# jackie840129/FedFR

Measured on AMD Instinct MI355X. Metric: images/sec (iresnet100+CosFace train step, bs=128/GPU, 112x112), higher is better.
Workload: dtype fp16; 1 GPU; iresnet100 + CosFace(s=30,m=0.4) + dense 1000-class cosine head, full train step (fwd+bwd+momentum-SGD), batch 128/GPU, 112x112 synthetic faces, random-init weights, fp16 activations/weights with fp32 accumulate + fp32 master weights, fp32 head; global_batch=128, parallelism=1 client per GPU (FedAvg), dp1, clients=1

## Files before the change

### fedfr_amd/csrc/gemm_nt_glds.hip

```cpp
#include "nt_epilogue.h"

#ifndef NT_GLDS_NS
#define NT_GLDS_NS 4
#endif
namespace {
template <int N_>
__device__ __forceinline__ void wait_vmcnt() {
  asm volatile("s_waitcnt vmcnt(%0)" ::"n"(N_) : "memory");
}

template <int BM, int BN, int WM, int WN, int NS, bool CONV>
__global__ __launch_bounds__(64 * WM * WN) void gemm_nt_glds_kernel(GemmNT p_) {
  GemmNT p = p_;
  if (p.par_on == 2) {
    const int cls = 3 - (int)blockIdx.z;
    p.par_h = cls >> 1; p.par_w = cls & 1;
    p.ksteps_total = (1 + p.par_h) * (1 + p.par_w) * p.cpt;
    p.ksteps_per_split = p.ksteps_total;
  }
  constexpr int NW = WM * WN, NT = 64 * NW;
  constexpr int TM = BM / WM / 16, TN = BN / WN / 16;
  constexpr int A_BYTES = BM * 128, B_BYTES = BN * 128, STAGE = A_BYTES + B_BYTES;
  constexpr int AP = (BM / 8) / NW, BP = (BN / 8) / NW, PER = AP + BP;
  constexpr int NRD = TM + TN, NM = TM * TN;
  static_assert((BM / 8) % NW == 0 && (BN / 8) % NW == 0 && NS >= 3 && NS <= 5 && AP >= 1 && BP >= 1, "tile geometry");
  typedef __attribute__((address_space(3))) void* lds_ptr_t;
  extern __shared__ __attribute__((aligned(1024))) unsigned char smem[];

  const int tid = threadIdx.x, lane = tid & 63;
  const int wave = __builtin_amdgcn_readfirstlane(tid >> 6);
  const int wm = wave / WN, wn = wave % WN;
  const int lid = xcd_remap(blockIdx.x, gridDim.x);
  const int bn = lid % p.nbn, bm = lid / p.nbn;
  const int split = blockIdx.y;
  const int m0 = bm * BM, n0 = bn * BN;
  const int kt0 = split * p.ksteps_per_split;
  const int kt1 = min(kt0 + p.ksteps_per_split, p.ksteps_total);

  const int prow = lane >> 3, pch = (lane & 7) ^ prow;
  constexpr unsigned OOB = 0xfffffff0u;
  int a_hb[AP], a_wb[AP];
  unsigned a_base[AP];
  bool a_ok[AP];
#pragma unroll
  for (int j = 0; j < AP; ++j) {
    const int m = m0 + (j * NW + wave) * 8 + prow;
    a_ok[j] = m < p.M;
    if (CONV) {
      const int mm = a_ok[j] ? m : 0;
      const int hw = p.Ho * p.Wo;
      const int img = mm / hw, rem = mm - img * hw;
      int ho = rem / p.Wo, wo = rem - ho * p.Wo;
      if (p.par_on) {
        ho = 2 * ho + p.par_h;
        wo = 2 * wo + p.par_w;
      }
      a_hb[j] = ho * p.stride - p.pad;
      a_wb[j] = wo * p.stride - p.pad;
      a_base[j] = ((unsigned)(img * p.H * p.W) * (unsigned)p.C + (unsigned)(pch * 8)) * 2u;
    } else {
      a_hb[j] = a_wb[j] = 0;
      a_base[j] = ((unsigned)(a_ok[j] ? m : 0) * (unsigned)p.lda + (unsigned)(pch * 8)) * 2u;
    }
  }
  unsigned b_base[BP];
  bool b_ok[BP];
#pragma unroll
  for (int j = 0; j < BP; ++j) {
    const int n = n0 + (j * NW + wave) * 8 + prow;
    b_ok[j] = n < p.N;
    b_base[j] = ((unsigned)(b_ok[j] ? n : 0) * (unsigned)p.K + (unsigned)(pch * 8)) * 2u;
  }
  int kti = kt0;
  int tap = kt0 / p.cpt, cc = kt0 - tap * p.cpt;
  int r = tap / p.S, s = tap - r * p.S;
  const int s0 = p.par_on ? 1 - p.par_w : 0, tstep = p.par_on ? 2 : 1;
  if (p.par_on) {
    const int nS = 1 + p.par_w;
    r = (1 - p.par_h) + 2 * (tap / nS);
    s = s0 + 2 * (tap % nS);
  }
  const __amdgpu_buffer_rsrc_t rsA = make_rsrc(p.A, p.a_bytes), rsB = make_rsrc(p.B, p.b_bytes);
  const int upm = p.up - 1, ups = p.up >> 1;
  const unsigned rowB = (unsigned)(p.W * p.C * 2), pixB = (unsigned)(p.C * 2);
  auto issue = [&](int slot) {
    unsigned char* sA = smem + slot * STAGE;
    unsigned char* sB = sA + A_BYTES;
    const bool live = kti < kt1;
    const unsigned kA = (unsigned)(CONV ? cc * 128 : kti * 128);
    const bool klive = live & (CONV | (kti * 64 + pch * 8 < p.K));
#pragma unroll
    for (int j = 0; j < AP; ++j) {
      bool ok = klive & a_ok[j];
      unsigned off = a_base[j] + kA;
      if (CONV) {
        int hp = a_hb[j] + r, wp = a_wb[j] + s;
        ok = ok & (((hp | wp) & upm) == 0);
        hp >>= ups;
        wp >>= ups;
        ok = ok & ((unsigned)hp < (unsigned)p.H) & ((unsigned)wp < (unsigned)p.W);
        off += __umul24((unsigned)hp, rowB) + __umul24((unsigned)wp, pixB);
      }
      __builtin_amdgcn_raw_ptr_buffer_load_lds(rsA, (lds_ptr_t)(sA + (j * NW + wave) * 1024), 16, (int)(ok ? off : OOB), 0, 0, 0);
    }
    const unsigned kB = (unsigned)(CONV ? ((r * p.S + s) * p.cpt + cc) * 128 : kti * 128);
#pragma unroll
    for (int j = 0; j < BP; ++j)
      __builtin_amdgcn_raw_ptr_buffer_load_lds(rsB, (lds_ptr_t)(sB + (j * NW + wave) * 1024), 16, (int)((klive & b_ok[j]) ? b_base[j] + kB : OOB), 0, 0, 0);
    ++kti;
    cc += 1;
    const bool wc = cc == p.cpt;
    cc = wc ? 0 : cc;
    s += wc ? tstep : 0;
    const bool ws = s >= p.S;
    s = ws ? s0 : s;
    r += ws ? tstep : 0;
  };

  const int l15 = lane & 15, lg = lane >> 4;
  int a_addr[TM], b_addr[TN];
#pragma unroll
  for (int mi = 0; mi < TM; ++mi) {
    const int row = wm * (BM / WM) + mi * 16 + l15;
    a_addr[mi] = row * 128 + ((lg ^ (row & 7)) << 4);
  }
#pragma unroll
  for (int ni = 0; ni < TN; ++ni) {
    const int row = wn * (BN / WN) + ni * 16 + l15;
    b_addr[ni] = A_BYTES + row * 128 + ((lg ^ (row & 7)) << 4);
  }
  f32x4_t acc[TN][TM];
#pragma unroll
  for (int a = 0; a < TN; ++a)
#pragma unroll
    for (int b = 0; b < TM; ++b) acc[a][b] = (f32x4_t){0.f, 0.f, 0.f, 0.f};
  bf16x8_t f0a[TM], f0b[TN], f1a[TM], f1b[TN];
  auto read_frags = [&](bf16x8_t (&fa)[TM], bf16x8_t (&fb)[TN], const unsigned char* st, int ks) {
#pragma unroll
    for (int ni = 0; ni < TN; ++ni) fb[ni] = *reinterpret_cast<const bf16x8_t*>(st + (b_addr[ni] ^ (ks * 64)));
#pragma unroll
    for (int mi = 0; mi < TM; ++mi) fa[mi] = *reinterpret_cast<const bf16x8_t*>(st + (a_addr[mi] ^ (ks * 64)));
  };
  auto mfma_all = [&](const bf16x8_t (&fa)[TM], const bf16x8_t (&fb)[TN]) {
#pragma unroll
    for (int ni = 0; ni < TN; ++ni)
#pragma unroll
      for (int mi = 0; mi < TM; ++mi) acc[ni][mi] = MFMA16(fb[ni], fa[mi], acc[ni][mi]);
  };

#pragma unroll
  for (int i = 0; i < NS - 1; ++i) issue(i);
  wait_vmcnt<(NS - 2) * PER>();
  __builtin_amdgcn_s_barrier();
  read_frags(f0a, f0b, smem, 0);
  int slot = 0;
  for (int kt = kt0; kt < kt1; ++kt) {
    const unsigned char* cur = smem + slot * STAGE;
    const int nslot = slot + 1 == NS ? 0 : slot + 1, fslot = slot == 0 ? NS - 1 : slot - 1;
    read_frags(f1a, f1b, cur, 1);
    mfma_all(f0a, f0b);
#pragma unroll
    for (int i = 0; i < NRD; ++i) {
      __builtin_amdgcn_sched_group_barrier(0x008, (NM / NRD) > 0 ? (NM / NRD) : 1, 0);
      __builtin_amdgcn_sched_group_barrier(0x100, 1, 0);
    }
    __builtin_amdgcn_sched_barrier(0);
    wait_vmcnt<(NS - 3) * PER>();
    __builtin_amdgcn_s_barrier();
    __builtin_amdgcn_sched_barrier(0);
    read_frags(f0a, f0b, smem + nslot * STAGE, 0);
    issue(fslot);
    mfma_all(f1a, f1b);
    constexpr int NE = NRD > PER ? NRD : PER, MP2 = (NM / NE) > 0 ? (NM / NE) : 1;
#pragma unroll
    for (int i = 0; i < NE; ++i) {
      __builtin_amdgcn_sched_group_barrier(0x008, MP2, 0);
      if (i < NRD) __builtin_amdgcn_sched_group_barrier(0x100, 1, 0);
      if (i < PER) __builtin_amdgcn_sched_group_barrier(0x020, 1, 0);
    }
    __builtin_amdgcn_sched_barrier(0);
    slot = nslot;
  }
  wait_vmcnt<0>();
  __syncthreads();
  nt_epilogue<BM, BN, WM, WN, NT>(p, acc, smem, bm, m0, n0, split, wm, wn, tid, lane);
}

template <int BM, int BN, int WM, int WN, int NS, bool CONV>
int launch_impl2(GemmNT p, int splits, int slot, hipStream_t st) {
  const int nbm = ceil_div(p.M, BM);
  p.nbn = ceil_div(p.N, BN);
  p.ksteps_per_split = ceil_div(p.ksteps_total, splits);
  FEDFR_REQUIRE(ceil_div(p.ksteps_total, p.ksteps_per_split) == splits, "gemm_nt_glds: splits=%d leaves an empty split (ksteps=%d)", splits,
                p.ksteps_total);
  constexpr size_t kRing = (size_t)NS * (BM + BN) * 128, kEpi = (size_t)BM * (BN * 2 + 16);
  constexpr size_t lds = kRing > kEpi ? kRing : kEpi;
  static PerDeviceOnce attr_once;
  attr_once.run([&] {
    hipFuncSetAttribute(reinterpret_cast<const void*>(&gemm_nt_glds_kernel<BM, BN, WM, WN, NS, CONV>), hipFuncAttributeMaxDynamicSharedMemorySize, (int)lds);
  });
  const dim3 grid(nbm * p.nbn, splits, p.par_on == 2 ? 4 : 1);
  ProfScope prof(slot, 2.0 * p.M * p.N * (p.par_on == 2 ? 64.0 * 9 * p.cpt : p.par_on ? 64.0 * p.ksteps_total : (double)p.K), st, gemm_nt_alg_bytes(p, splits));
  hipLaunchKernelGGL((gemm_nt_glds_kernel<BM, BN, WM, WN, NS, CONV>), grid, dim3(64 * WM * WN), lds, st, p);
  FEDFR_LAUNCH_CHECK("gemm_nt_glds");
  return FEDFR_OK;
}
template <int BM, int BN, int WM, int WN, int NS>
int launch_impl(const GemmNT& p, int splits, int slot, hipStream_t st) {
  if (p.mode == 1) {
    FEDFR_REQUIRE((long long)p.W * p.C * 2 < (1 << 24) && p.H < (1 << 15), "gemm_nt_glds: image row too large for the 24-bit address multiplies");
    return launch_impl2<BM, BN, WM, WN, NS, true>(p, splits, slot, st);
  }
  return launch_impl2<BM, BN, WM, WN, NS, false>(p, splits, slot, st);
}
}

int g_nt_glds = 4;

bool gemm_nt_glds_applies(const GemmNT& p, int BM, int splits) {
  const bool pays = (g_nt_glds & 8) || (!p.par_on && ceil_div(p.ksteps_total, splits) >= 16);
  return (g_nt_glds & 7) > 0 && p.N > 64 && (BM == 128 || BM == 64) && pays && !p.bpart && !p.esc && !p.eadd && !p.Cb2;
}

int launch_nt_glds(const GemmNT& p, int BM, int splits, int slot, hipStream_t st) {
  FEDFR_REQUIRE(gemm_nt_glds_applies(p, BM, splits), "gemm_nt_glds: unsupported problem");
  const int v = g_nt_glds & 7;
  const bool up = v >= 3 && BM == 64 && (!p.stats || ceil_div(p.M, 64) == 2 * ceil_div(p.M, 128));
  if (BM == 128 || up) return (v & 1) == 0 ? launch_impl<128, 128, 2, 4, NT_GLDS_NS>(p, splits, slot, st) : launch_impl<128, 128, 2, 2, 4>(p, splits, slot, st);
  return launch_impl<64, 128, 1, 4, 3>(p, splits, slot, st);
}
```

Measured before the change: 8402 images/sec.

## Hoist implicit-GEMM conv gather address math to once per filter tap

Adds a tap-stepped variant of the conv gather GEMM kernel, templated on channel-chunks-per-tap (1,2,4,8). Per-row spatial coordinates and validity are computed once, and the per-tap voffset and validity are recomputed only when the filter tap advances. Between tap changes each k-step just adds the chunk offset, which removes integer address arithmetic and predicate work from the inner loop. The cost is more template instantiations and extra registers held across the loop, which could lower occupancy.

Measured after the change: 8423 images/sec, median of 6. About the same (+0.2%).

```diff
diff --git a/fedfr_amd/csrc/gemm_nt_glds.hip b/fedfr_amd/csrc/gemm_nt_glds.hip
--- a/fedfr_amd/csrc/gemm_nt_glds.hip
+++ b/fedfr_amd/csrc/gemm_nt_glds.hip
@@ -1,7 +1,11 @@
 #include "nt_epilogue.h"
+#include "nt_gather_plan.h"
 
 #ifndef NT_GLDS_NS
 #define NT_GLDS_NS 4
+#endif
+#ifndef NT_GLDS_TAPSTEP
+#define NT_GLDS_TAPSTEP 1
 #endif
 namespace {
 template <int N_>
@@ -9,8 +13,9 @@
   asm volatile("s_waitcnt vmcnt(%0)" ::"n"(N_) : "memory");
 }
 
-template <int BM, int BN, int WM, int WN, int NS, bool CONV>
+template <int BM, int BN, int WM, int WN, int NS, bool CONV, int CPT>
 __global__ __launch_bounds__(64 * WM * WN) void gemm_nt_glds_kernel(GemmNT p_) {
+  static_assert(CPT == 0 || CONV, "the tap-stepped plan is the conv gather's");
   GemmNT p = p_;
   if (p.par_on == 2) {
     const int cls = 3 - (int)blockIdx.z;
@@ -116,6 +121,39 @@
     s = ws ? s0 : s;
     r += ws ? tstep : 0;
   };
+  const NtPlanGeom pg = nt_plan_geom(p.H, p.W, p.C, p.S, p.up, p.cpt, p.par_on, p.par_w);
+  NtPlanRow prw[AP];
+  unsigned voff_tap[AP], kB_tap = 0;
+  bool ok_tap[AP];
+  auto plan_tap = [&]() {
+#pragma unroll
+    for (int j = 0; j < AP; ++j) nt_plan_tap(pg, prw[j], r, s, voff_tap[j], ok_tap[j]);
+    kB_tap = nt_plan_weight_tap(pg, r, s);
+  };
+  if constexpr (CPT > 0) {
+#pragma unroll
+    for (int j = 0; j < AP; ++j)
+      prw[j] = nt_plan_row(m0 + (j * NW + wave) * 8 + prow, p.M, p.Ho, p.Wo, p.H, p.W, p.C, p.stride, p.pad, p.par_on, p.par_h, p.par_w, pch);
+    nt_plan_tap_first(pg, p.par_on, p.par_h, p.par_w, kt0 / CPT, r, s);
+    plan_tap();
+  }
+  auto issue_tap = [&](int slot, int ci) {
+    unsigned char* sA = smem + slot * STAGE;
+    unsigned char* sB = sA + A_BYTES;
+    const bool live = kti < kt1;
+#pragma unroll
+    for (int j = 0; j < AP; ++j)
+      __builtin_amdgcn_raw_ptr_buffer_load_lds(rsA, (lds_ptr_t)(sA + (j * NW + wave) * 1024), 16, (int)nt_plan_voffset(voff_tap[j], ok_tap[j], live, ci), 0, 0, 0);
+    const unsigned kB = kB_tap + (unsigned)ci * 128u;
+#pragma unroll
+    for (int j = 0; j < BP; ++j)
+      __builtin_amdgcn_raw_ptr_buffer_load_lds(rsB, (lds_ptr_t)(sB + (j * NW + wave) * 1024), 16, (int)((live & b_ok[j]) ? b_base[j] + kB : OOB), 0, 0, 0);
+    ++kti;
+    if (ci == CPT - 1) {
+      nt_plan_tap_next(pg, r, s);
+      plan_tap();
+    }
+  };
 
   const int l15 = lane & 15, lg = lane >> 4;
   int a_addr[TM], b_addr[TN];
@@ -149,12 +187,15 @@
   };
 
 #pragma unroll
-  for (int i = 0; i < NS - 1; ++i) issue(i);
+  for (int i = 0; i < NS - 1; ++i) {
+    if constexpr (CPT > 0) issue_tap(i, i % CPT);
+    else issue(i);
+  }
   wait_vmcnt<(NS - 2) * PER>();
   __builtin_amdgcn_s_barrier();
   read_frags(f0a, f0b, smem, 0);
   int slot = 0;
-  for (int kt = kt0; kt < kt1; ++kt) {
+  auto kstep = [&](auto&& issue_next) {
     const unsigned char* cur = smem + slot * STAGE;
     const int nslot = slot + 1 == NS ? 0 : slot + 1, fslot = slot == 0 ? NS - 1 : slot - 1;
     read_frags(f1a, f1b, cur, 1);
@@ -169,7 +210,7 @@
     __builtin_amdgcn_s_barrier();
     __builtin_amdgcn_sched_barrier(0);
     read_frags(f0a, f0b, smem + nslot * STAGE, 0);
-    issue(fslot);
+    issue_next(fslot);
     mfma_all(f1a, f1b);
     constexpr int NE = NRD > PER ? NRD : PER, MP2 = (NM / NE) > 0 ? (NM / NE) : 1;
 #pragma unroll
@@ -180,12 +221,34 @@
     }
     __builtin_amdgcn_sched_barrier(0);
     slot = nslot;
+  };
+  if constexpr (CPT > 0) {
+    for (int kt = kt0; kt < kt1; kt += CPT) {
+#pragma unroll
+      for (int u = 0; u < CPT; ++u) kstep([&](int fslot) { issue_tap(fslot, (u + NS - 1) % CPT); });
+    }
+  } else {
+    for (int kt = kt0; kt < kt1; ++kt) kstep([&](int fslot) { issue(fslot); });
   }
   wait_vmcnt<0>();
   __syncthreads();
   nt_epilogue<BM, BN, WM, WN, NT>(p, acc, smem, bm, m0, n0, split, wm, wn, tid, lane);
 }
 
+template <int BM, int BN, int WM, int WN, int NS, bool CONV, int CPT>
+int launch_kernel(const GemmNT& p, int nbm, int splits, int slot, hipStream_t st) {
+  constexpr size_t kRing = (size_t)NS * (BM + BN) * 128, kEpi = (size_t)BM * (BN * 2 + 16);
+  constexpr size_t lds = kRing > kEpi ? kRing : kEpi;
+  static PerDeviceOnce attr_once;
+  attr_once.run([&] {
+    hipFuncSetAttribute(reinterpret_cast<const void*>(&gemm_nt_glds_kernel<BM, BN, WM, WN, NS, CONV, CPT>), hipFuncAttributeMaxDynamicSharedMemorySize, (int)lds);
+  });
+  const dim3 grid(nbm * p.nbn, splits, p.par_on == 2 ? 4 : 1);
+  ProfScope prof(slot, 2.0 * p.M * p.N * (p.par_on == 2 ? 64.0 * 9 * p.cpt : p.par_on ? 64.0 * p.ksteps_total : (double)p.K), st, gemm_nt_alg_bytes(p, splits));
+  hipLaunchKernelGGL((gemm_nt_glds_kernel<BM, BN, WM, WN, NS, CONV, CPT>), grid, dim3(64 * WM * WN), lds, st, p);
+  FEDFR_LAUNCH_CHECK("gemm_nt_glds");
+  return FEDFR_OK;
+}
 template <int BM, int BN, int WM, int WN, int NS, bool CONV>
 int launch_impl2(GemmNT p, int splits, int slot, hipStream_t st) {
   const int nbm = ceil_div(p.M, BM);
@@ -193,17 +256,16 @@
   p.ksteps_per_split = ceil_div(p.ksteps_total, splits);
   FEDFR_REQUIRE(ceil_div(p.ksteps_total, p.ksteps_per_split) == splits, "gemm_nt_glds: splits=%d leaves an empty split (ksteps=%d)", splits,
                 p.ksteps_total);
-  constexpr size_t kRing = (size_t)NS * (BM + BN) * 128, kEpi = (size_t)BM * (BN * 2 + 16);
-  constexpr size_t lds = kRing > kEpi ? kRing : kEpi;
-  static PerDeviceOnce attr_once;
-  attr_once.run([&] {
-    hipFuncSetAttribute(reinterpret_cast<const void*>(&gemm_nt_glds_kernel<BM, BN, WM, WN, NS, CONV>), hipFuncAttributeMaxDynamicSharedMemorySize, (int)lds);
-  });
-  const dim3 grid(nbm * p.nbn, splits, p.par_on == 2 ? 4 : 1);
-  ProfScope prof(slot, 2.0 * p.M * p.N * (p.par_on == 2 ? 64.0 * 9 * p.cpt : p.par_on ? 64.0 * p.ksteps_total : (double)p.K), st, gemm_nt_alg_bytes(p, splits));
-  hipLaunchKernelGGL((gemm_nt_glds_kernel<BM, BN, WM, WN, NS, CONV>), grid, dim3(64 * WM * WN), lds, st, p);
-  FEDFR_LAUNCH_CHECK("gemm_nt_glds");
-  return FEDFR_OK;
+  if constexpr (CONV && NT_GLDS_TAPSTEP) {
+    if (p.ksteps_per_split % p.cpt == 0) switch (p.cpt) {
+        case 1: return launch_kernel<BM, BN, WM, WN, NS, true, 1>(p, nbm, splits, slot, st);
+        case 2: return launch_kernel<BM, BN, WM, WN, NS, true, 2>(p, nbm, splits, slot, st);
+        case 4: return launch_kernel<BM, BN, WM, WN, NS, true, 4>(p, nbm, splits, slot, st);
+        case 8: return launch_kernel<BM, BN, WM, WN, NS, true, 8>(p, nbm, splits, slot, st);
+        default: break;
+      }
+  }
+  return launch_kernel<BM, BN, WM, WN, NS, CONV, 0>(p, nbm, splits, slot, st);
 }
 template <int BM, int BN, int WM, int WN, int NS>
 int launch_impl(const GemmNT& p, int splits, int slot, hipStream_t st) {
diff --git a/fedfr_amd/csrc/nt_gather_plan.h b/fedfr_amd/csrc/nt_gather_plan.h
--- /dev/null
+++ b/fedfr_amd/csrc/nt_gather_plan.h
@@ -0,0 +1,92 @@
+#pragma once
+
+#if defined(__HIPCC__)
+#define NT_PLAN_FN __host__ __device__ __forceinline__
+#else
+#define NT_PLAN_FN inline
+#endif
+
+constexpr unsigned NT_PLAN_OOB = 0xfffffff0u;
+
+NT_PLAN_FN unsigned nt_plan_mul24(unsigned a, unsigned b) {
+#if defined(__HIP_DEVICE_COMPILE__)
+  return __umul24(a, b);
+#else
+  return (a & 0xffffffu) * (b & 0xffffffu);
+#endif
+}
+
+struct NtPlanGeom {
+  int H, W, S;
+  int upm, ups;
+  unsigned rowB, pixB;
+  int s0, tstep;
+  unsigned tapB;
+};
+
+NT_PLAN_FN NtPlanGeom nt_plan_geom(int H, int W, int C, int S, int up, int cpt, int par_on, int par_w) {
+  NtPlanGeom g;
+  g.H = H; g.W = W; g.S = S;
+  g.upm = up - 1; g.ups = up >> 1;
+  g.rowB = (unsigned)(W * C * 2); g.pixB = (unsigned)(C * 2);
+  g.s0 = par_on ? 1 - par_w : 0; g.tstep = par_on ? 2 : 1;
+  g.tapB = (unsigned)cpt * 128u;
+  return g;
+}
+
+struct NtPlanRow {
+  int hb, wb;
+  unsigned base;
+  bool ok;
+};
+
+NT_PLAN_FN NtPlanRow nt_plan_row(int m, int M, int Ho, int Wo, int H, int W, int C, int stride, int pad, int par_on, int par_h, int par_w, int pch) {
+  NtPlanRow row;
+  row.ok = m < M;
+  const int mm = row.ok ? m : 0;
+  const int hw = Ho * Wo;
+  const int img = mm / hw, rem = mm - img * hw;
+  int ho = rem / Wo, wo = rem - ho * Wo;
+  if (par_on) {
+    ho = 2 * ho + par_h;
+    wo = 2 * wo + par_w;
+  }
+  row.hb = ho * stride - pad;
+  row.wb = wo * stride - pad;
+  row.base = ((unsigned)(img * H * W) * (unsigned)C + (unsigned)(pch * 8)) * 2u;
+  return row;
+}
+
+NT_PLAN_FN void nt_plan_tap_first(const NtPlanGeom& g, int par_on, int par_h, int par_w, int tap, int& r, int& s) {
+  if (par_on) {
+    const int nS = 1 + par_w;
+    r = (1 - par_h) + 2 * (tap / nS);
+    s = g.s0 + 2 * (tap % nS);
+  } else {
+    r = tap / g.S;
+    s = tap - r * g.S;
+  }
+}
+
+NT_PLAN_FN void nt_plan_tap_next(const NtPlanGeom& g, int& r, int& s) {
+  s += g.tstep;
+  const bool ws = s >= g.S;
+  s = ws ? g.s0 : s;
+  r += ws ? g.tstep : 0;
+}
+
+NT_PLAN_FN void nt_plan_tap(const NtPlanGeom& g, const NtPlanRow& row, int r, int s, unsigned& voff, bool& ok) {
+  int hp = row.hb + r, wp = row.wb + s;
+  bool v = row.ok & (((hp | wp) & g.upm) == 0);
+  hp >>= g.ups;
+  wp >>= g.ups;
+  v = v & ((unsigned)hp < (unsigned)g.H) & ((unsigned)wp < (unsigned)g.W);
+  voff = row.base + nt_plan_mul24((unsigned)hp, g.rowB) + nt_plan_mul24((unsigned)wp, g.pixB);
+  ok = v;
+}
+
+NT_PLAN_FN unsigned nt_plan_voffset(unsigned voff_tap, bool ok_tap, bool live, int cc) {
+  return (live & ok_tap) ? voff_tap + (unsigned)cc * 128u : NT_PLAN_OOB;
+}
+
+NT_PLAN_FN unsigned nt_plan_weight_tap(const NtPlanGeom& g, int r, int s) { return (unsigned)(r * g.S + s) * g.tapB; }
```
